# jwcalder/GraphLearningLayer

Measured on AMD Instinct MI355X. Metric: GLL fwd+bwd calls/sec (base=500,batch=500,d=512,k=10) at 1/2/4/8 GPU, higher is better.
Workload: dtype f32; 1 GPU; ns; base=500, batch=500, d=512, k=10, classes=10, parallelism=dp1, upstream_grad=fixed seeded dL/dU, autograd_thread=caller, collective=none

## Files before the change

graphlearninglayer_amd/_lib.py:

```python
from __future__ import annotations

import ctypes as ct
import os
import threading

HERE = os.path.dirname(os.path.abspath(__file__))
LIB_PATH = os.environ.get("GLL_LIB_PATH") or os.path.join(HERE, "libgll.so")

GLL_OK = 0
GLL_DT_F32, GLL_DT_F64, GLL_DT_I64 = 0, 1, 2
FLAG_CG_GRID = 1
FLAG_CG_PERCOL = 8
FLAG_DIAG_GRID_OVERSUB = 128
FLAG_DIAG_GRID_FAIL = 256
FLAG_CG_ELL = 512
FLAG_CG_VR = 1024
FLAG_GRAD_ROWS = 2048
FLAG_GRAD_CHUNK = 4096
FLAG_GRAM_INLINE = 8192
FLAG_BWD_UNFUSED = 16384
FLAG_KNN_PANEL = 65536
FLAG_D2_F32 = 131072
FLAG_ROW_ORDER_OFF = 262144
KNOB_VR_RV, KNOB_GRID_CAP, KNOB_GRAM_TILE, KNOB_SEL_FORM, KNOB_GRAM_TAIL, KNOB_ROW_PRE = 0, 1, 2, 3, 4, 5
ST_TINY_EPS, ST_FWD_NONCONV, ST_FWD_ITERS, ST_BWD_NONCONV, ST_BWD_ITERS = 0, 1, 2, 3, 4
ST_KNN_RESCAN = 5
ST_SOLVE_FAILED = 6
ST_GRID_RESCUED = 10
ST_KNN_MERGE = 7
ST_NWORDS = 16
K_GRAM, K_SELECT, K_FINALIZE, K_CG, K_EDGE, K_GRAD = range(6)
K_BWD = 6
K_PARAM = 7
K_LOSS = 8
K_COUNT = 9
PG_Y, PG_TAU, PG_EPS = 1, 2, 4
XT_F32, XT_F16, XT_BF16 = 0, 1, 2
UF_NORMALIZE = 1
MAX_D_FEATURES = 4096

EXPORTS = (
    "gll_workspace_bytes", "gll_forward", "gll_backward", "gll_forward_batched",
    "gll_backward_batched", "gll_param_grad_scratch_bytes", "gll_param_grad_batched",
    "gll_ce_head_scratch_bytes", "gll_ce_head_batched", "gll_margin_head_scratch_bytes",
    "gll_margin_head_batched", "gll_graph", "gll_workspace_view",
    "gll_cg_csr_workspace_bytes", "gll_cg_csr", "gll_prof_enable", "gll_prof_read",
    "gll_kernel_name", "gll_strerror", "gll_set_knob", "gll_build_id", "gll_select_route",
    "gll_workspace_solve_view", "gll_workspace_knn_view", "gll_gram_route",
    "gll_features_forward", "gll_features_backward", "gll_features_calls",
)


class Problem(ct.Structure):
    _fields_ = [
        ("n", ct.c_int32), ("d", ct.c_int32), ("base", ct.c_int32), ("C", ct.c_int32),
        ("K", ct.c_int32), ("max_iter", ct.c_int32), ("tau", ct.c_float), ("eps", ct.c_float),
        ("rtol", ct.c_float), ("flags", ct.c_int32), ("status_sink", ct.c_void_p),
    ]


class View(ct.Structure):
    _fields_ = [(name, ct.c_void_p) for name in (
        "knn_idx", "knn_d2", "eps", "row_start", "row_len", "col", "w", "d2", "deg", "U32",
        "wadj", "status")]
# ... 52 lines not shown
    lib.gll_workspace_knn_view.restype = i32
    lib.gll_gram_route.argtypes = [P, i32, i32, i32, ct.POINTER(ct.c_int32)]
    lib.gll_gram_route.restype = i32
    lib.gll_cg_csr_workspace_bytes.argtypes = [i32, i32]
    lib.gll_cg_csr_workspace_bytes.restype = sz
    lib.gll_cg_csr.argtypes = [i32, i32, vp, vp, vp, vp, vp, ct.c_float, i32, vp, vp, vp, vp]
    lib.gll_cg_csr.restype = i32
    lib.gll_prof_enable.argtypes = [i32, i32]
    lib.gll_prof_enable.restype = i32
    lib.gll_prof_read.argtypes = [i32, ct.POINTER(ct.c_double), ct.POINTER(ct.c_int)]
    lib.gll_prof_read.restype = i32
    lib.gll_kernel_name.argtypes = [i32]
    lib.gll_kernel_name.restype = ct.c_char_p
    lib.gll_select_route.argtypes = [ct.POINTER(Problem), i32, i32, i32, ct.POINTER(ct.c_int32)]
    lib.gll_select_route.restype = i32
    lib.gll_set_knob.argtypes = [i32, i32]
    lib.gll_set_knob.restype = i32
    lib.gll_strerror.argtypes = [i32]
    lib.gll_strerror.restype = ct.c_char_p
    lib.gll_build_id.argtypes = []
    lib.gll_build_id.restype = ct.c_char_p
    lib.gll_features_forward.argtypes = [ct.c_int64, ct.c_int32, vp, i32, i32, vp, vp, vp]
    lib.gll_features_forward.restype = i32
    lib.gll_features_backward.argtypes = [ct.c_int64, ct.c_int32, vp, vp, vp, i32, vp, i32, vp]
    lib.gll_features_backward.restype = i32
    lib.gll_features_calls.argtypes = []
    lib.gll_features_calls.restype = ct.c_int64
    return lib


# ... 39 lines not shown
```

graphlearninglayer_amd/csrc/api.hip:

```cpp
#include <atomic>
#include <cstdio>
#include <cstdlib>
#include <mutex>
#include <unordered_map>
#include <vector>

#include "knn_route.h"

namespace gll {

struct ProfState {
    int period[GLL_K_COUNT] = {};
    long count[GLL_K_COUNT] = {};
    bool on[GLL_K_COUNT] = {};
    std::vector<hipEvent_t> pending[GLL_K_COUNT];
    std::vector<hipEvent_t> pool;
    std::mutex mu;
    hipEvent_t get() {
        if (!pool.empty()) {
            hipEvent_t e = pool.back();
            pool.pop_back();
            return e;
        }
        hipEvent_t e;
// ... 202 lines not shown
    if (B < 1 || B > 65535) return GLL_ERR_INVALID_ARG;
    if (!X || !ws || !gradX || (p->n > p->base && !gbar)) return GLL_ERR_INVALID_ARG;
    if (g_dtype != GLL_DT_F32 && g_dtype != GLL_DT_F64) return GLL_ERR_INVALID_ARG;
    Layout L(*p);
    const Batch bt = make_batch(p, L, B, GLL_DT_F32, g_dtype);
    hipStream_t s = static_cast<hipStream_t>(stream);
    const float rtol = p->rtol > 0.f ? p->rtol : 1e-6f;
    const int max_iter = p->max_iter > 0 ? p->max_iter : 1000;
    int32_t* st = public_status(p, L, ws);
    float* wU = L.at<float>(ws, L.Wadj) + size_t(L.base) * L.C;
    const bool auto_eps = !(p->eps > 0.f);
    if (B == 1 && !auto_eps) {
        const hipError_t e = launch_cg_grad_fused(L, ws, gbar, g_dtype, X, p->eps, gradX, rtol,
                                                  max_iter, st + GLL_ST_BWD_NONCONV,
                                                  st + GLL_ST_BWD_ITERS, st + GLL_ST_SOLVE_FAILED,
                                                  vec_ok(X, p->d), s);
        if (e != hipErrorNotSupported) return hip_status(e);
    }
    hipError_t e = launch_cg_luu(L, bt, ws, gbar, bt.g, g_dtype, nullptr, wU, rtol, max_iter,
                                 st + GLL_ST_BWD_NONCONV, st + GLL_ST_BWD_ITERS,
                                 st + GLL_ST_SOLVE_FAILED, s);
    if (e != hipSuccess) return GLL_ERR_HIP;
    return hip_status(launch_backward_grad(L, bt, ws, X, auto_eps, p->eps, gradX,
                                           vec_ok(X, p->d), s));
}

}

using namespace gll;

extern "C" {
// ... 279 lines not shown
    if (rc != GLL_OK) return rc;
    if (B < 1 || B > 65535 || !out) return GLL_ERR_INVALID_ARG;
    Layout L(*p);
    if (L.PR < L.n ? (B > 1 || rows < 1 || rows > L.PR) : rows != L.n) return GLL_ERR_INVALID_ARG;
    Batch bt;
    bt.B = B;
    const SelRoute rt = select_route(L, bt, x_aligned && p->d % 4 == 0, 0, rows);
    const SelVariant& v = rt.v;
    const SelWideVariant& w = rt.w;
    const int32_t words[GLL_SEL_ROUTE_WORDS] = {
        rt.wide, rt.wide ? w.V : v.KC, rt.wide ? w.NP : v.V, rt.wide ? w.CAP : v.NP,
        rt.wide ? w.KMX : v.PG, rt.wide ? w.TOP : v.NU, v.XQ, v.R, v.CH, v.H,
        select_table_index(rt), select_table_rows()};
    for (int q = 0; q < GLL_SEL_ROUTE_WORDS; ++q) out[q] = words[q];
    return words[10] >= 0 ? GLL_OK : GLL_ERR_UNSUPPORTED;
}

#ifndef GLL_BUILD_ID
#define GLL_BUILD_ID "unknown"
#endif
const char* gll_build_id(void) { return GLL_BUILD_ID; }

const char* gll_strerror(int code) {
    switch (code) {
        case GLL_OK: return "ok";
        case GLL_ERR_INVALID_ARG: return "invalid argument";
        case GLL_ERR_UNSUPPORTED: return "unsupported problem size (see include/gll.h limits)";
        case GLL_ERR_HIP: return "HIP launch error";
        default: return "unknown error";
    }
// ... 69 lines not shown
```

graphlearninglayer_amd/csrc/gll_internal.h:

```cpp
#pragma once

#include <hip/hip_runtime.h>
#include <hip/hip_ext.h>
#include <stdint.h>
#include <stdlib.h>

#include <type_traits>

#include "gll.h"

namespace gll {

constexpr int kWave = 64;
constexpr int kMaxKm1 = 56;
constexpr int kMaxKm1Wide = 128;
constexpr int kMaxKm1Huge = 256;

constexpr int kStOvfCount = 8;
constexpr int kStBump = 9;
constexpr int kStPermValid = 11;
constexpr int kPiv = 64;
constexpr int kStWords = GLL_ST_NWORDS;

inline int ell_slots(int m) {
// ... 450 lines not shown
                              int max_iter, int32_t* st_nonconv, int32_t* st_iters,
                              int32_t* st_failed, hipStream_t s);
hipError_t launch_cg_grid_csr(int m, int C, const int32_t* row_ptr, const int32_t* col,
                              const float* val, int64_t nnz, const float* b, float* x,
                              float atol, int max_iter, int32_t* iters, int32_t* nonconv,
                              int32_t* failed, float* ws, hipStream_t s);
hipError_t launch_cg_csr(int m, int C, const int32_t* row_ptr, const int32_t* col,
                         const float* val, const float* b, float* x, float atol, int max_iter,
                         int32_t* iters, int32_t* nonconv, float* gvec, hipStream_t s);
hipError_t launch_backward_grad(const Layout& L, const Batch& bt, void* ws, const float* X,
                                bool auto_eps, float eps_fixed, float* gradX, bool vec,
                                hipStream_t s);
hipError_t launch_cg_grad_fused(const Layout& L, void* ws, const void* gbar, int g_dtype,
                                const float* X, float eps_fixed, float* gradX, float rtol,
                                int max_iter, int32_t* st_nonconv, int32_t* st_iters,
                                int32_t* st_failed, bool vec, hipStream_t s);
size_t param_grad_scratch_bytes(int n, int B);
hipError_t launch_param_grad(const Layout& L, int B, void* ws, float eps_fixed, int what,
                             float* gradY, double* grad_tau, double* grad_eps, void* scratch,
                             hipStream_t s);
size_t ce_head_scratch_bytes(int m, int B);
hipError_t launch_ce_head(const Layout& L, int B, void* ws, const int64_t* targets, double* loss,
                          float* gbar, double* row_loss, int64_t* pred_label, int64_t* correct,
                          void* scratch, hipStream_t s);
hipError_t launch_margin_head(const Layout& L, int B, void* ws, const int64_t* other, double* loss,
                              float* gbar, double* row_margin, int64_t* label, int64_t* second,
                              int64_t* moved, void* scratch, hipStream_t s);
hipError_t launch_unit_rows(int64_t rows, int d, const void* Z, int z_dtype, int flags, float* X,
                            float* rnorm, hipStream_t s);
hipError_t launch_unit_grad(int64_t rows, int d, const float* gX, const float* X,
                            const float* rnorm, int flags, void* gZ, int z_dtype, hipStream_t s);
// ... 4 lines not shown
```

graphlearninglayer_amd/csrc/solve.hip:

```cpp
#include <cstdio>
#include <cstdlib>
#include <mutex>
#include <unordered_set>

#include "gll_internal.h"
#include "grad_common.h"

namespace gll {

GLL_TRACE_UNIT(solve)
#ifdef GLL_TRACE
static __device__ unsigned long long g_fz[5 * 4096];
void trace_read_fz(unsigned long long* out) {
    (void)hipMemcpyFromSymbol(out, HIP_SYMBOL(g_fz), sizeof(g_fz));
}
#define GLL_FZ(slot, wv, val)                                                                  \
    do {                                                                                       \
        if (lane_id() == 0 && (wv) < 4096) g_fz[(slot) * 4096 + (wv)] = (val);                 \
    } while (0)
#else
#define GLL_FZ(slot, wv, val) do {} while (0)
#endif

static constexpr size_t kLdsLimit = 160 * 1024;
// ... 844 lines not shown
    if (cap > eu_bound) cap = eu_bound;
    if (cap > kOvfLds) cap = kOvfLds;
    if (cap < 0) cap = 0;
    lds += size_t(cap) * 8;
    if (S > ell_emit(L, bt.B)) return hipErrorInvalidValue;
    auto fn = cg_ell_kernel<NT, R, S, TB, MODE>;
    allow_full_lds(reinterpret_cast<const void*>(fn));
    launch_k(fn, dim3(L.C, bt.B), NT, lds, s,
        L.m, L.C, L.base, L.at<int32_t>(ws, L.row_start), L.at<int32_t>(ws, L.row_len),
        L.at<int32_t>(ws, L.ucnt), L.at<int32_t>(ws, L.col), L.at<float>(ws, L.w),
        L.at<float>(ws, L.diag), b, out64, out32, rtol, max_iter, int(cap), st_nonconv, st_iters,
        L.at<int4>(ws, L.ell), bt.ws, bs, bt.u, bt.st);
    return launch_status("solve.hip:run_ell");
}

struct EllCgArgs {
    int m, C, base;
    const int32_t* row_start;
    const int32_t* row_len;
    const int32_t* ucnt;
    const int32_t* col;
    const float* wv;
    const float* diag;
    const void* b;
    float* out32;
    float rtol;
    int max_iter, mat_cap;
    int32_t* st_nonconv;
    int32_t* st_iters;
    const int4* ell;
};

template <int NT, int S, typename TB, int ND>
__global__ __launch_bounds__(NT) void cg_grad_fused_kernel(EllCgArgs c, EdgeArgs a,
                                                           const float* __restrict__ X,
                                                           float* __restrict__ out,
                                                           unsigned* fsync, int32_t* st_failed) {
    const int C = c.C;
    if (int(blockIdx.x) < C) {
        cg_ell_body<NT, 1, S, TB, 3>(int2{int(blockIdx.x), 0}, fsync, c.m, C, c.base,
                                     c.row_start, c.row_len, c.ucnt, c.col, c.wv, c.diag,
                                     static_cast<const TB*>(c.b), nullptr, c.out32, c.rtol,
                                     c.max_iter, c.mat_cap, c.st_nonconv, c.st_iters, c.ell,
                                     0, 0, 0, 0);
        return;
    }
    constexpr int NC = 10;
    constexpr int EB = ND <= 2 ? 16 : 8;
    __shared__ int s_ok;
    const int lane = lane_id();
    int i0;
    {
        extern __shared__ __attribute__((aligned(16))) float smem[];
        int* srt = reinterpret_cast<int*>(smem);
        int* crk = srt + a.n;
        const int nch = (a.n + kWave - 1) / kWave;
        int* cnt = crk + a.n;
        constexpr int NW = NT / kWave;
        const int w = threadIdx.x >> 6;
        for (int q = w; q < nch; q += NW) {
            const int i = q * kWave + lane;
            int cls = -1;
            if (i < a.n) {
                float bv = -3.0e38f;
                cls = 0;
#pragma unroll
// ... 19 lines not shown
            for (int kk = 0; kk < k; ++kk)
                for (int q = 0; q < nch; ++q) before += cnt[q * NC + kk];
            for (int q = 0; q < nch; ++q) {
                const int c0 = cnt[q * NC + k];
                cnt[q * NC + k] = before;
                before += c0;
            }
        }
        __syncthreads();
        for (int i = threadIdx.x; i < a.n; i += NT) {
            const int v = crk[i];
            srt[cnt[(i / kWave) * NC + (v >> 16)] + (v & 0xffff)] = i;
        }
        __syncthreads();
        const int G = int(gridDim.x) - C, b = int(blockIdx.x), x = b & 7;
        int ord = 0;
#pragma unroll
        for (int xx = 0; xx < 8; ++xx) {
            const int f = C + ((xx - C % 8 + 8) & 7);
            const int cx = f < C + G ? (C + G - 1 - f) / 8 + 1 : 0;
            if (xx < x) ord += cx;
        }
        ord += (b - (C + ((x - C % 8 + 8) & 7))) >> 3;
        const int pos = ord * NW + w;
        i0 = pos < a.n ? srt[pos] : a.n;
    }
    const bool live = i0 < a.n;
    const int i = live ? i0 : 0;
    const int d = a.d;
    const int beg = a.row_start[i];
    const int end = live ? beg + a.row_len[i] : beg;
    const float ei = a.eps_fixed;
    const float* xi = X + size_t(i) * d;
    f32x4 xv[ND];
#pragma unroll
    for (int q = 0; q < ND; ++q) xv[q] = load4_raw<true>(xi, 4 * lane + 4 * kWave * q, d);
    typedef float f32x2 __attribute__((ext_vector_type(2)));
    float pi[NC];
#pragma unroll
    for (int q = 0; q < NC; q += 2) {
        const f32x2 v = *reinterpret_cast<const f32x2*>(a.P + size_t(i) * NC + q);
        pi[q] = v.x, pi[q + 1] = v.y;
    }
    const __amdgpu_buffer_rsrc_t rw =
        __builtin_amdgcn_make_buffer_rsrc(const_cast<float*>(a.Wadj), 0, a.n * NC * 4, 0x00020000);
    auto edge_pre = [&](int e, int& cj, float& we, float* pj) {
        const bool el = e < end;
        cj = el ? a.col[e] : i;
        we = el ? a.w[e] : 0.f;
#pragma unroll
        for (int q = 0; q < NC; q += 2) {
            const f32x2 v = *reinterpret_cast<const f32x2*>(a.P + size_t(cj) * NC + q);
// ... 10 lines not shown
        float g = 0.f;
#pragma unroll
        for (int q = 0; q < NC; ++q) g = __builtin_fmaf(wi[q] - wj[q], pj[q] - pi[q], g);
        const float ej = a.eps_fixed;
        const float v = -8.f * we / (ei * ej);
        return e < end ? g * v : 0.f;
    };
    int cj;
    float we, pj[NC];
    edge_pre(beg + lane, cj, we, pj);
    const int cnt0 = min(kWave, end - beg);
#ifdef GLL_TRACE
    const bool tr = int(blockIdx.x) == C && threadIdx.x == 0;
    if (tr) g_trace[16] = __builtin_amdgcn_s_memrealtime();
#endif
    f32x4 v[EB][ND];
#pragma unroll
    for (int u = 0; u < EB; ++u) {
        const int t = u < cnt0 ? u : 0;
        const float* xj = X + size_t(readlane_i(cj, t)) * d;
#pragma unroll
        for (int q = 0; q < ND; ++q) v[u][q] = load4_raw<true>(xj, 4 * lane + 4 * kWave * q, d);
    }
    if (threadIdx.x == 0) {
        int ok = __hip_atomic_load(fsync + 64, __ATOMIC_RELAXED, __HIP_MEMORY_SCOPE_AGENT) == 0u;
        unsigned spins = 0;
        const unsigned long long t0 = wall_ticks();
        while (ok && __hip_atomic_load(fsync + 96, __ATOMIC_RELAXED, __HIP_MEMORY_SCOPE_AGENT) ==
               0u) {
            __builtin_amdgcn_s_sleep(2);
            if ((++spins & 15u) == 0 && wall_ticks() - t0 > kWaitTicks) {
                ok = 0;
                break;
            }
        }
        s_ok = ok;
    }
    __syncthreads();
    const bool ok = s_ok != 0;
#ifdef GLL_TRACE
    if (tr) g_trace[17] = __builtin_amdgcn_s_memrealtime();
    GLL_FZ(0, i0, __builtin_amdgcn_s_memrealtime());
#endif
#pragma unroll
    for (int q = 0; q < NC; ++q)
        wi[q] = __builtin_bit_cast(
            float, __builtin_amdgcn_raw_buffer_load_b32(rw, (i * NC + q) * 4, 0, kSc1W));
    f32x4 acc[ND];
#pragma unroll
    for (int q = 0; q < ND; ++q) acc[q] = f32x4{0.f, 0.f, 0.f, 0.f};
    for (int e0 = beg; e0 < end; e0 += kWave) {
        if (e0 != beg) edge_pre(e0 + lane, cj, we, pj);
        const float cf = edge_coef(e0 + lane, cj, we, pj);
#ifdef GLL_TRACE
        if (e0 == beg) {
            float cfo = cf;
            asm volatile("s_waitcnt vmcnt(0)" : "+v"(cfo)::"memory");
            if (cfo == 12345.f) g_trace[9] = 0;
            GLL_FZ(1, i0, __builtin_amdgcn_s_memrealtime());
        }
#endif
        const int cnt = min(kWave, end - e0);
        for (int t0 = 0; t0 < cnt; t0 += EB) {
            float sv[EB];
            if (e0 != beg || t0 != 0) {
#pragma unroll
                for (int u = 0; u < EB; ++u) {
                    const int t = t0 + u < cnt ? t0 + u : t0;
                    const float* xj = X + size_t(readlane_i(cj, t)) * d;
#pragma unroll
                    for (int q = 0; q < ND; ++q) v[u][q] = load4_raw<true>(xj, 4 * lane + 4 * kWave * q, d);
                }
            }
#pragma unroll
            for (int u = 0; u < EB; ++u) {
                const int t = t0 + u < cnt ? t0 + u : t0;
                sv[u] = t0 + u < cnt ? readlane_f(cf, t) : 0.f;
            }
#pragma unroll
            for (int u = 0; u < EB; ++u) {
#pragma unroll
                for (int q = 0; q < ND; ++q) acc[q] += sv[u] * (xv[q] - v[u][q]);
            }
        }
    }
#ifdef GLL_TRACE
    {
        f32x4 ao = acc[0];
        asm volatile("" : "+v"(ao));
        if (ao.x == 12345.f) g_trace[9] = 0;
        GLL_FZ(2, i0, __builtin_amdgcn_s_memrealtime());
    }
#endif
    if (live) {
        const float nanf_ = __builtin_nanf("");
        float* oi = out + size_t(i) * d;
#pragma unroll
        for (int q = 0; q < ND; ++q) {
            const int k = 4 * lane + 4 * kWave * q;
            const f32x4 r = ok ? acc[q] : f32x4{nanf_, nanf_, nanf_, nanf_};
            if (k < d) __builtin_nontemporal_store(r, reinterpret_cast<f32x4*>(oi + k));
        }
    }
#ifdef GLL_TRACE
    asm volatile("s_waitcnt vmcnt(0)" ::: "memory");
    GLL_FZ(3, i0, __builtin_amdgcn_s_memrealtime());
    {
        unsigned hw;
        asm volatile("s_getreg_b32 %0, hwreg(HW_REG_HW_ID)" : "=s"(hw));
        unsigned xcc;
        asm volatile("s_getreg_b32 %0, hwreg(HW_REG_XCC_ID)" : "=s"(xcc));
        GLL_FZ(4, i0, (unsigned long long)(end - beg) | ((unsigned long long)((hw >> 8) & 0xffff) << 16) |
                          ((unsigned long long)(xcc & 0xff) << 40));
    }
#endif
    __syncthreads();
#ifdef GLL_TRACE
    if (tr) g_trace[18] = __builtin_amdgcn_s_memrealtime();
    if (threadIdx.x == 0) atomicMax(&g_trace[19], __builtin_amdgcn_s_memrealtime());
#endif
    if (threadIdx.x == 0) {
        if (!ok) {
            __hip_atomic_fetch_or(fsync + 64, 1u, __ATOMIC_RELAXED, __HIP_MEMORY_SCOPE_AGENT);
            if (st_failed) atomicOr(st_failed, 1);
            asm volatile("s_waitcnt vmcnt(0)" ::: "memory");
        }
        const unsigned ng = gridDim.x - unsigned(C);
        const unsigned old = __hip_atomic_fetch_add(fsync + 32, 1u, __ATOMIC_RELAXED,
                                                    __HIP_MEMORY_SCOPE_AGENT);
        if (old + 1u == ng &&
            __hip_atomic_load(fsync + 64, __ATOMIC_RELAXED, __HIP_MEMORY_SCOPE_AGENT) == 0u) {
            __hip_atomic_store(fsync, 0u, __ATOMIC_RELAXED, __HIP_MEMORY_SCOPE_AGENT);
            __hip_atomic_store(fsync + 32, 0u, __ATOMIC_RELAXED, __HIP_MEMORY_SCOPE_AGENT);
            __hip_atomic_store(fsync + 96, 0u, __ATOMIC_RELAXED, __HIP_MEMORY_SCOPE_AGENT);
        }
    }
}

template <int NT, int ND, typename TB>
static hipError_t run_fused(const Layout& L, void* ws, const TB* b, const float* X,
                            float eps_fixed, float* gradX, float rtol, int max_iter,
                            int32_t* st_nonconv, int32_t* st_iters, int32_t* st_failed,
                            hipStream_t s) {
    constexpr int S = 24;
    size_t lds = 128 * 4 + size_t((L.m + 3) & ~3) * 4 * 2;
    const int64_t eu_bound = int64_t(L.m + L.n) * (L.K - 1);
    int64_t cap = int64_t(kLdsDyn - lds) / 8;
    if (cap > eu_bound) cap = eu_bound;
    if (cap < 0) cap = 0;
    lds += size_t(cap) * 8;
    const size_t sort_lds = size_t(L.n) * 8 + size_t((L.n + kWave - 1) / kWave) * 10 * 4;
    if (sort_lds > kLdsDyn) return hipErrorNotSupported;
    if (lds < sort_lds) lds = sort_lds;
    auto fn = cg_grad_fused_kernel<NT, S, TB, ND>;
    allow_full_lds(reinterpret_cast<const void*>(fn));
    const int G = L.C + (L.n + NT / kWave - 1) / (NT / kWave);
    const int nb = occupancy_blocks(reinterpret_cast<const void*>(fn), NT, lds);
    if (int64_t(nb) * device_cus() < G) return hipErrorNotSupported;
    EllCgArgs c;
    c.m = L.m;
    c.C = L.C;
    c.base = L.base;
    c.row_start = L.at<int32_t>(ws, L.row_start);
    c.row_len = L.at<int32_t>(ws, L.row_len);
    c.ucnt = L.at<int32_t>(ws, L.ucnt);
    c.col = L.at<int32_t>(ws, L.col);
    c.wv = L.at<float>(ws, L.w);
    c.diag = L.at<float>(ws, L.diag);
    c.b = b;
    c.out32 = L.at<float>(ws, L.Wadj) + size_t(L.base) * L.C;
    c.rtol = rtol;
    c.max_iter = max_iter;
    c.mat_cap = int(cap);
    c.st_nonconv = st_nonconv;
    c.st_iters = st_iters;
    c.ell = L.at<int4>(ws, L.ell);
    const EdgeArgs a = make_edge_args(L, 0, ws, eps_fixed);
    prof_begin(GLL_K_BWD, s);
    launch_k(fn, dim3(unsigned(G)), NT, lds, s, c, a, X, gradX, L.at<unsigned>(ws, L.fsync),
             st_failed);
    prof_end(GLL_K_BWD, s);
    return launch_status("solve.hip:run_fused");
}

hipError_t launch_cg_grad_fused(const Layout& L, void* ws, const void* gbar, int g_dtype,
                                const float* X, float eps_fixed, float* gradX, float rtol,
                                int max_iter, int32_t* st_nonconv, int32_t* st_iters,
                                int32_t* st_failed, bool vec, hipStream_t s) {
    const int m = L.m;
    if (L.C != 10 || !(eps_fixed > 0.f) || !vec || m < 1 || m > 512 || L.RV != 0 ||
        ell_emit(L, 1) != 24 || L.d > 1024)
        return hipErrorNotSupported;
    if (L.flags & (GLL_FLAG_BWD_UNFUSED | GLL_FLAG_CG_GRID | GLL_FLAG_GRAD_CHUNK))
        return hipErrorNotSupported;
    if (size_t(L.n) * L.d * 4 > (size_t(4) << 20)) return hipErrorNotSupported;
    const int nd = (L.d + 255) / 256;
#define GLL_FUSED(NT_)                                                                       \
    {                                                                                        \
        if (g_dtype == GLL_DT_F32) {                                                         \
            const float* b = static_cast<const float*>(gbar);                                \
            if (nd <= 1) return run_fused<NT_, 1>(L, ws, b, X, eps_fixed, gradX, rtol, max_iter, st_nonconv, st_iters, st_failed, s); \
            if (nd <= 2) return run_fused<NT_, 2>(L, ws, b, X, eps_fixed, gradX, rtol, max_iter, st_nonconv, st_iters, st_failed, s); \
            return run_fused<NT_, 4>(L, ws, b, X, eps_fixed, gradX, rtol, max_iter, st_nonconv, st_iters, st_failed, s); \
        }                                                                                    \
        const double* b = static_cast<const double*>(gbar);                                  \
        if (nd <= 1) return run_fused<NT_, 1>(L, ws, b, X, eps_fixed, gradX, rtol, max_iter, st_nonconv, st_iters, st_failed, s); \
        if (nd <= 2) return run_fused<NT_, 2>(L, ws, b, X, eps_fixed, gradX, rtol, max_iter, st_nonconv, st_iters, st_failed, s); \
        return run_fused<NT_, 4>(L, ws, b, X, eps_fixed, gradX, rtol, max_iter, st_nonconv, st_iters, st_failed, s); \
    }
    if (m <= 64) GLL_FUSED(64);
    if (m <= 128) GLL_FUSED(128);
    if (m <= 256) GLL_FUSED(256);
    GLL_FUSED(512);
#undef GLL_FUSED
}

template <int NT, int R, int RV, typename TB>
static hipError_t run_vr(const Layout& L, const Batch& bt, void* ws, const TB* b, size_t bs,
                         double* out64, float* out32, float rtol, int max_iter,
                         int32_t* st_nonconv, int32_t* st_iters, hipStream_t s) {
    if (L.m > NT * R || L.RV != RV || L.VRM <= 0 || L.VRM > 63) {
        (void)hipGetLastError();
        return hipErrorInvalidValue;
    }
    const size_t mp4 = size_t((L.m + 3) & ~3);
    const size_t lds = 128 * 4 + mp4 * 4 + (size_t(NT) * RV + 4 * mp4) * 4 +
                       size_t(NT) * RV * 4 + mp4 * 4;
// ... 170 lines not shown
```

include/gll.h:

```cpp
#ifndef GLL_H
#define GLL_H

#include <stddef.h>
#include <stdint.h>

#ifdef __cplusplus
extern "C" {
#endif

#define GLL_OK 0
#define GLL_ERR_INVALID_ARG (-1)
#define GLL_ERR_UNSUPPORTED (-2)
#define GLL_ERR_HIP (-3)

#define GLL_DT_F32 0
#define GLL_DT_F64 1
#define GLL_DT_I64 2

#define GLL_ST_TINY_EPS 0
#define GLL_ST_FWD_NONCONV 1
#define GLL_ST_FWD_ITERS 2
#define GLL_ST_BWD_NONCONV 3
#define GLL_ST_BWD_ITERS 4
#define GLL_ST_KNN_RESCAN 5
#define GLL_ST_SOLVE_FAILED 6
#define GLL_ST_KNN_MERGE 7
#define GLL_ST_GRID_RESCUED 10
#define GLL_ST_NWORDS 16

#define GLL_FLAG_CG_GRID 1
#define GLL_FLAG_CG_PERCOL 8
#define GLL_FLAG_DIAG_GRID_OVERSUB 128
#define GLL_FLAG_DIAG_GRID_FAIL 256
#define GLL_FLAG_CG_ELL 512
#define GLL_FLAG_CG_VR 1024
#define GLL_FLAG_GRAD_ROWS 2048
#define GLL_FLAG_GRAD_CHUNK 4096
#define GLL_FLAG_GRAM_INLINE 8192
#define GLL_FLAG_BWD_UNFUSED 16384
#define GLL_FLAG_KNN_PANEL 65536
#define GLL_FLAG_D2_F32 131072
#define GLL_FLAG_ROW_ORDER_OFF 262144
#define GLL_FLAG_ALL (1 | 8 | 128 | 256 | 512 | 1024 | 2048 | 4096 | 8192 | 16384 | 65536 | \
                      131072 | 262144)

#define GLL_KNOB_VR_RV 0
#define GLL_KNOB_GRID_CAP 1
#define GLL_KNOB_GRAM_TILE 2
#define GLL_KNOB_SEL_FORM 3
#define GLL_KNOB_GRAM_TAIL 4
#define GLL_KNOB_ROW_PRE 5
#define GLL_KNOB_COUNT 6
int gll_set_knob(int knob, int value);

typedef struct gll_problem {
    int32_t n;
    int32_t d;
    int32_t base;
    int32_t C;
    int32_t K;
    int32_t max_iter;
    float tau;
    float eps;
    float rtol;
    int32_t flags;
    int32_t* status_sink;
} gll_problem;
// ... 96 lines not shown
#define GLL_K_CG 3
#define GLL_K_EDGE 4
#define GLL_K_GRAD 5
#define GLL_K_BWD 6
#define GLL_K_PARAM 7
#define GLL_K_LOSS 8
#define GLL_K_COUNT 9
int gll_prof_enable(int kid, int period);
int gll_prof_read(int kid, double* ms_total, int* count);
const char* gll_kernel_name(int kid);

#define GLL_SEL_ROUTE_WORDS 12
int gll_select_route(const gll_problem* p, int B, int x_aligned, int rows,
                     int32_t out[GLL_SEL_ROUTE_WORDS]);

const char* gll_build_id(void);

const char* gll_strerror(int code);

#define GLL_XT_F32 0
#define GLL_XT_F16 1
#define GLL_XT_BF16 2
#define GLL_UF_NORMALIZE 1
int gll_features_forward(int64_t rows, int32_t d, const void* Z, int z_dtype, int flags,
                         float* X, float* rnorm, void* stream);
int gll_features_backward(int64_t rows, int32_t d, const float* gX, const float* X,
                          const float* rnorm, int flags, void* gZ, int z_dtype, void* stream);
int64_t gll_features_calls(void);

#ifdef __cplusplus
// ... 4 lines not shown
```

Before: 16230 calls/s.

## Split long gradient rows across multiple waves in fused CG-grad kernel

The fused CG+gradient kernel can now split a row's feature dimension into 2 or 4 parts when the row has many edges, so one row is handled by several waves. The grid grows (up to twice the row count) to supply those waves, with a prefix-sum assignment of work items to waves. Extra waves exit early through a counter that keeps the sync-reset logic working. The aim is better load balance and more memory-level parallelism for the edge gather. The cost is larger launches, more prefix-scan work per block, and duplicated per-row coefficient work.

```diff
diff --git a/graphlearninglayer_amd/_lib.py b/graphlearninglayer_amd/_lib.py
--- a/graphlearninglayer_amd/_lib.py
+++ b/graphlearninglayer_amd/_lib.py
@@ -23,11 +23,13 @@
 FLAG_D2_F32 = 131072
 FLAG_ROW_ORDER_OFF = 262144
 KNOB_VR_RV, KNOB_GRID_CAP, KNOB_GRAM_TILE, KNOB_SEL_FORM, KNOB_GRAM_TAIL, KNOB_ROW_PRE = 0, 1, 2, 3, 4, 5
+KNOB_GRAD_SPLIT = 6
 ST_TINY_EPS, ST_FWD_NONCONV, ST_FWD_ITERS, ST_BWD_NONCONV, ST_BWD_ITERS = 0, 1, 2, 3, 4
 ST_KNN_RESCAN = 5
 ST_SOLVE_FAILED = 6
 ST_GRID_RESCUED = 10
 ST_KNN_MERGE = 7
+ST_GRAD_SPLIT = 12
 ST_NWORDS = 16
 K_GRAM, K_SELECT, K_FINALIZE, K_CG, K_EDGE, K_GRAD = range(6)
 K_BWD = 6
@@ -47,7 +49,7 @@
     "gll_cg_csr_workspace_bytes", "gll_cg_csr", "gll_prof_enable", "gll_prof_read",
     "gll_kernel_name", "gll_strerror", "gll_set_knob", "gll_build_id", "gll_select_route",
     "gll_workspace_solve_view", "gll_workspace_knn_view", "gll_gram_route",
-    "gll_features_forward", "gll_features_backward", "gll_features_calls",
+    "gll_features_forward", "gll_features_backward", "gll_features_calls", "gll_fused_plan",
 )
 
 
@@ -130,6 +132,8 @@
     lib.gll_kernel_name.restype = ct.c_char_p
     lib.gll_select_route.argtypes = [ct.POINTER(Problem), i32, i32, i32, ct.POINTER(ct.c_int32)]
     lib.gll_select_route.restype = i32
+    lib.gll_fused_plan.argtypes = [ct.POINTER(Problem), i32, i32, ct.POINTER(ct.c_int32)]
+    lib.gll_fused_plan.restype = i32
     lib.gll_set_knob.argtypes = [i32, i32]
     lib.gll_set_knob.restype = i32
     lib.gll_strerror.argtypes = [i32]
diff --git a/graphlearninglayer_amd/csrc/api.hip b/graphlearninglayer_amd/csrc/api.hip
--- a/graphlearninglayer_amd/csrc/api.hip
+++ b/graphlearninglayer_amd/csrc/api.hip
@@ -240,7 +240,7 @@
         const hipError_t e = launch_cg_grad_fused(L, ws, gbar, g_dtype, X, p->eps, gradX, rtol,
                                                   max_iter, st + GLL_ST_BWD_NONCONV,
                                                   st + GLL_ST_BWD_ITERS, st + GLL_ST_SOLVE_FAILED,
-                                                  vec_ok(X, p->d), s);
+                                                  st + GLL_ST_GRAD_SPLIT, vec_ok(X, p->d), s);
         if (e != hipErrorNotSupported) return hip_status(e);
     }
     hipError_t e = launch_cg_luu(L, bt, ws, gbar, bt.g, g_dtype, nullptr, wU, rtol, max_iter,
@@ -550,6 +550,19 @@
         select_table_index(rt), select_table_rows()};
     for (int q = 0; q < GLL_SEL_ROUTE_WORDS; ++q) out[q] = words[q];
     return words[10] >= 0 ? GLL_OK : GLL_ERR_UNSUPPORTED;
+}
+
+int gll_fused_plan(const gll_problem* p, int x_aligned, int capacity,
+                   int32_t out[GLL_FUSED_PLAN_WORDS]) {
+    int rc = check(p);
+    if (rc != GLL_OK) return rc;
+    if (!out) return GLL_ERR_INVALID_ARG;
+    Layout L(*p);
+    if (capacity < 0)
+        return fused_plan_device(L, p->eps, x_aligned && p->d % 4 == 0, GLL_DT_F64, out)
+                   ? GLL_OK : GLL_ERR_UNSUPPORTED;
+    return fused_plan(L, p->eps, x_aligned && p->d % 4 == 0, capacity, out) ? GLL_OK
+                                                                             : GLL_ERR_UNSUPPORTED;
 }
 
 #ifndef GLL_BUILD_ID
diff --git a/graphlearninglayer_amd/csrc/gll_internal.h b/graphlearninglayer_amd/csrc/gll_internal.h
--- a/graphlearninglayer_amd/csrc/gll_internal.h
+++ b/graphlearninglayer_amd/csrc/gll_internal.h
@@ -488,7 +488,9 @@
 hipError_t launch_cg_grad_fused(const Layout& L, void* ws, const void* gbar, int g_dtype,
                                 const float* X, float eps_fixed, float* gradX, float rtol,
                                 int max_iter, int32_t* st_nonconv, int32_t* st_iters,
-                                int32_t* st_failed, bool vec, hipStream_t s);
+                                int32_t* st_failed, int32_t* st_split, bool vec, hipStream_t s);
+bool fused_plan(const Layout& L, float eps_fixed, bool vec, int64_t capacity, int32_t out[8]);
+bool fused_plan_device(const Layout& L, float eps_fixed, bool vec, int g_dtype, int32_t out[8]);
 size_t param_grad_scratch_bytes(int n, int B);
 hipError_t launch_param_grad(const Layout& L, int B, void* ws, float eps_fixed, int what,
                              float* gradY, double* grad_tau, double* grad_eps, void* scratch,
diff --git a/graphlearninglayer_amd/csrc/solve.hip b/graphlearninglayer_amd/csrc/solve.hip
--- a/graphlearninglayer_amd/csrc/solve.hip
+++ b/graphlearninglayer_amd/csrc/solve.hip
@@ -882,6 +882,69 @@
     return launch_status("solve.hip:run_ell");
 }
 
+struct FusedPlan {
+    int nt, nd;
+    int grid;
+    int base_grid;
+    int waves;
+    int split;
+    size_t lds;
+    int64_t mat_cap;
+};
+
+__host__ __device__ inline int row_parts(int len, int eb, int pmax) {
+    const int l = len < kWave ? len : kWave;
+    int p = 1;
+    while (p < pmax && l > eb * p) p *= 2;
+    return p;
+}
+__host__ __device__ constexpr int max_parts(int nd) { return nd >= 2 ? 4 : 1; }
+__host__ __device__ constexpr int fused_eb(int nd) { return nd <= 2 ? 16 : 8; }
+
+template <int W> struct PartVec { typedef f32x4 type; };
+template <> struct PartVec<2> { typedef f32x2 type; };
+template <int W>
+__device__ __forceinline__ typename PartVec<W>::type part_load(const float* __restrict__ p, int k,
+                                                               int lim) {
+    return *reinterpret_cast<const typename PartVec<W>::type*>(p + (k < lim ? k : 0));
+}
+template <int NV, int W>
+__device__ __forceinline__ void part_load_row(typename PartVec<W>::type* r,
+                                              const float* __restrict__ x, int fo, int lane, int d) {
+#pragma unroll
+    for (int q = 0; q < NV; ++q) r[q] = part_load<W>(x, fo + W * lane + W * kWave * q, d);
+}
+
+template <int S, int NV, int W>
+__device__ __forceinline__ void part_gather(typename PartVec<W>::type* v,
+                                            const float* __restrict__ X, int cj, int t0, int cnt,
+                                            int fo, int lane, int d) {
+#pragma unroll
+    for (int u = 0; u < S; ++u) {
+        const int t = t0 + u < cnt ? t0 + u : t0;
+        part_load_row<NV, W>(v + u * NV, X + size_t(readlane_i(cj, t)) * d, fo, lane, d);
+    }
+}
+
+template <int S, int NV, int W, bool FIRST>
+__device__ __forceinline__ void part_fma(typename PartVec<W>::type* acc,
+                                         const typename PartVec<W>::type* xv,
+                                         const typename PartVec<W>::type* v, float cf, int t0) {
+    static_assert(kWave % S == 0, "slots divide the 64 edges of a pass");
+    constexpr int SB = S < 16 ? S : 16;
+#pragma unroll
+    for (int u0 = 0; u0 < S; u0 += SB) {
+        float sv[SB];
+#pragma unroll
+        for (int u = 0; u < SB; ++u) sv[u] = readlane_f(cf, FIRST ? u0 + u : t0 + u0 + u);
+#pragma unroll
+        for (int u = 0; u < SB; ++u) {
+#pragma unroll
+            for (int q = 0; q < NV; ++q) acc[q] += sv[u] * (xv[q] - v[(u0 + u) * NV + q]);
+        }
+    }
+}
+
 struct EllCgArgs {
     int m, C, base;
     const int32_t* row_start;
@@ -903,7 +966,8 @@
 __global__ __launch_bounds__(NT) void cg_grad_fused_kernel(EllCgArgs c, EdgeArgs a,
                                                            const float* __restrict__ X,
                                                            float* __restrict__ out,
-                                                           unsigned* fsync, int32_t* st_failed) {
+                                                           unsigned* fsync, int32_t* st_failed,
+                                                           int32_t* st_split, int split) {
     const int C = c.C;
     if (int(blockIdx.x) < C) {
         cg_ell_body<NT, 1, S, TB, 3>(int2{int(blockIdx.x), 0}, fsync, c.m, C, c.base,
@@ -917,7 +981,20 @@
     constexpr int EB = ND <= 2 ? 16 : 8;
     __shared__ int s_ok;
     const int lane = lane_id();
-    int i0;
+    auto exit_count = [&]() {
+        const unsigned ng = gridDim.x - unsigned(C);
+        const unsigned old = __hip_atomic_fetch_add(fsync + 32, 1u, __ATOMIC_RELAXED,
+                                                    __HIP_MEMORY_SCOPE_AGENT);
+        if (old + 1u == ng &&
+            __hip_atomic_load(fsync + 64, __ATOMIC_RELAXED, __HIP_MEMORY_SCOPE_AGENT) == 0u) {
+            __hip_atomic_store(fsync, 0u, __ATOMIC_RELAXED, __HIP_MEMORY_SCOPE_AGENT);
+            __hip_atomic_store(fsync + 32, 0u, __ATOMIC_RELAXED, __HIP_MEMORY_SCOPE_AGENT);
+            __hip_atomic_store(fsync + 96, 0u, __ATOMIC_RELAXED, __HIP_MEMORY_SCOPE_AGENT);
+        }
+    };
+    constexpr int PMAX = max_parts(ND);
+    int i0, pos;
+    int part = 0, nparts = 1;
     {
         extern __shared__ __attribute__((aligned(16))) float smem[];
         int* srt = reinterpret_cast<int*>(smem);
@@ -967,16 +1044,87 @@
         }
         __syncthreads();
         const int G = int(gridDim.x) - C, b = int(blockIdx.x), x = b & 7;
-        int ord = 0;
-#pragma unroll
-        for (int xx = 0; xx < 8; ++xx) {
-            const int f = C + ((xx - C % 8 + 8) & 7);
-            const int cx = f < C + G ? (C + G - 1 - f) / 8 + 1 : 0;
-            if (xx < x) ord += cx;
-        }
-        ord += (b - (C + ((x - C % 8 + 8) & 7))) >> 3;
-        const int pos = ord * NW + w;
+        auto xcd_rank = [&](int act) -> int {
+            const int j = (b - (C + ((x - C % 8 + 8) & 7))) >> 3;
+            int ord = 0, all = 0, tot = 0, mine = 0;
+#pragma unroll
+            for (int xx = 0; xx < 8; ++xx) {
+                const int f = C + ((xx - C % 8 + 8) & 7);
+                const int cx = f < C + G ? (C + G - 1 - f) / 8 + 1 : 0;
+                const int ax = min(cx, act / 8 + (xx < act % 8 ? 1 : 0));
+                if (xx < x) ord += ax, all += cx;
+                if (xx == x) mine = ax;
+                tot += ax;
+            }
+            if (tot < act) return all + j;
+            return j < mine ? ord + j : -1;
+        };
+        pos = xcd_rank(G) * NW + w;
         i0 = pos < a.n ? srt[pos] : a.n;
+        int nsplit = 0;
+        int wrank = 0;
+        if (PMAX > 1 && split) {
+            int* ipre = crk;
+            int* coff = cnt;
+            for (int q = w; q < nch; q += NW) {
+                const int r = q * kWave + lane;
+                const int p = r < a.n ? row_parts(a.row_len[srt[r]], EB, PMAX) : 0;
+                int inc = p;
+#pragma unroll
+                for (int off = 1; off < kWave; off <<= 1) {
+                    const int t = __shfl_up(inc, off);
+                    if (lane >= off) inc += t;
+                }
+                if (r < a.n) ipre[r] = ((inc - p) << 3) | p;
+                const uint64_t ms = __ballot(p > 1);
+                if (lane == kWave - 1) coff[q] = inc, coff[nch + q] = __popcll(ms);
+            }
+            __syncthreads();
+            if (threadIdx.x == 0) {
+                int items = 0, rows = 0;
+                for (int q = 0; q < nch; ++q) {
+                    const int c0 = coff[q];
+                    coff[q] = items;
+                    items += c0;
+                    rows += coff[nch + q];
+                }
+                coff[2 * nch] = items;
+                coff[2 * nch + 1] = rows;
+            }
+            __syncthreads();
+            const int items = coff[2 * nch];
+            if (items <= G * NW) {
+                nsplit = coff[2 * nch + 1];
+                i0 = a.n;
+                wrank = xcd_rank((items + NW - 1) / NW);
+                pos = wrank * NW + w;
+                if (wrank >= 0 && pos < items) {
+                    int cq = 0;
+                    for (int q0 = 0; q0 < nch; q0 += kWave) {
+                        const int q = q0 + lane;
+                        cq += __popcll(__ballot(q < nch && coff[q] <= pos));
+                    }
+                    const int r = (cq - 1) * kWave + lane;
+                    const int e = r < a.n ? ipre[r] : 0;
+                    const int first = coff[cq - 1] + (e >> 3);
+                    const uint64_t hit = __ballot((e & 7) != 0 && pos >= first && pos < first + (e & 7));
+                    if (hit != 0) {
+                        const int l = __ffsll((unsigned long long)hit) - 1;
+                        i0 = srt[(cq - 1) * kWave + l];
+                        nparts = readlane_i(e & 7, l);
+                        part = pos - readlane_i(first, l);
+                    }
+                }
+            }
+        }
+        if (int(blockIdx.x) == C && threadIdx.x == 0 && st_split) *st_split = nsplit;
+        if (wrank < 0) {
+            if (threadIdx.x == 0) exit_count();
+            return;
+        }
+        nparts = __builtin_amdgcn_readfirstlane(nparts);
+        part = __builtin_amdgcn_readfirstlane(part);
+        i0 = __builtin_amdgcn_readfirstlane(i0);
     }
     const bool live = i0 < a.n;
     const int i = live ? i0 : 0;
@@ -985,10 +1133,16 @@
     const int end = live ? beg + a.row_len[i] : beg;
     const float ei = a.eps_fixed;
     const float* xi = X + size_t(i) * d;
-    f32x4 xv[ND];
-#pragma unroll
-    for (int q = 0; q < ND; ++q) xv[q] = load4_raw<true>(xi, 4 * lane + 4 * kWave * q, d);
-    typedef float f32x2 __attribute__((ext_vector_type(2)));
+    const int fo = part * (4 * kWave * ND / nparts);
+    auto by_part = [&](auto f) {
+        if constexpr (PMAX > 1) {
+            if (nparts == 2) return f(std::integral_constant<int, ND / 2>{}, std::integral_constant<int, 4>{});
+            if (nparts == 4)
+                return f(std::integral_constant<int, (ND >= 4 ? ND / 4 : 1)>{},
+                         std::integral_constant<int, (ND >= 4 ? 4 : 2)>{});
+        }
+        return f(std::integral_constant<int, ND>{}, std::integral_constant<int, 4>{});
+    };
     float pi[NC];
 #pragma unroll
     for (int q = 0; q < NC; q += 2) {
@@ -1029,106 +1183,98 @@
     const bool tr = int(blockIdx.x) == C && threadIdx.x == 0;
     if (tr) g_trace[16] = __builtin_amdgcn_s_memrealtime();
 #endif
-    f32x4 v[EB][ND];
-#pragma unroll
-    for (int u = 0; u < EB; ++u) {
-        const int t = u < cnt0 ? u : 0;
-        const float* xj = X + size_t(readlane_i(cj, t)) * d;
-#pragma unroll
-        for (int q = 0; q < ND; ++q) v[u][q] = load4_raw<true>(xj, 4 * lane + 4 * kWave * q, d);
-    }
-    if (threadIdx.x == 0) {
-        int ok = __hip_atomic_load(fsync + 64, __ATOMIC_RELAXED, __HIP_MEMORY_SCOPE_AGENT) == 0u;
-        unsigned spins = 0;
-        const unsigned long long t0 = wall_ticks();
-        while (ok && __hip_atomic_load(fsync + 96, __ATOMIC_RELAXED, __HIP_MEMORY_SCOPE_AGENT) ==
-               0u) {
-            __builtin_amdgcn_s_sleep(2);
-            if ((++spins & 15u) == 0 && wall_ticks() - t0 > kWaitTicks) {
-                ok = 0;
-                break;
-            }
-        }
-        s_ok = ok;
-    }
-    __syncthreads();
-    const bool ok = s_ok != 0;
+    auto wait_release = [&]() -> bool {
+        if (threadIdx.x == 0) {
+            int ok = __hip_atomic_load(fsync + 64, __ATOMIC_RELAXED, __HIP_MEMORY_SCOPE_AGENT) == 0u;
+            unsigned spins = 0;
+            const unsigned long long t0 = wall_ticks();
+            while (ok && __hip_atomic_load(fsync + 96, __ATOMIC_RELAXED,
+                                           __HIP_MEMORY_SCOPE_AGENT) == 0u) {
+                __builtin_amdgcn_s_sleep(2);
+                if ((++spins & 15u) == 0 && wall_ticks() - t0 > kWaitTicks) {
+                    ok = 0;
+                    break;
+                }
+            }
+            s_ok = ok;
+        }
+        __syncthreads();
+        return s_ok != 0;
+    };
+    bool ok = false;
+    if (!live) ok = wait_release();
+    else by_part([&](auto nv, auto wd) {
+        constexpr int NV = nv(), W = wd();
+        constexpr int SL = EB * ND * 4 / (NV * W);
+        typedef typename PartVec<W>::type VT;
+        VT xv[NV];
+        part_load_row<NV, W>(xv, xi, fo, lane, d);
+        VT v[SL * NV];
+        part_gather<SL, NV, W>(v, X, cj, 0, cnt0, fo, lane, d);
+        ok = wait_release();
 #ifdef GLL_TRACE
-    if (tr) g_trace[17] = __builtin_amdgcn_s_memrealtime();
-    GLL_FZ(0, i0, __builtin_amdgcn_s_memrealtime());
+        if (tr) g_trace[17] = __builtin_amdgcn_s_memrealtime();
+        const int fzi = live ? pos : 4096;
+        GLL_FZ(0, fzi, __builtin_amdgcn_s_memrealtime());
 #endif
 #pragma unroll
-    for (int q = 0; q < NC; ++q)
-        wi[q] = __builtin_bit_cast(
-            float, __builtin_amdgcn_raw_buffer_load_b32(rw, (i * NC + q) * 4, 0, kSc1W));
-    f32x4 acc[ND];
-#pragma unroll
-    for (int q = 0; q < ND; ++q) acc[q] = f32x4{0.f, 0.f, 0.f, 0.f};
-    for (int e0 = beg; e0 < end; e0 += kWave) {
-        if (e0 != beg) edge_pre(e0 + lane, cj, we, pj);
-        const float cf = edge_coef(e0 + lane, cj, we, pj);
+        for (int q = 0; q < NC; ++q)
+            wi[q] = __builtin_bit_cast(
+                float, __builtin_amdgcn_raw_buffer_load_b32(rw, (i * NC + q) * 4, 0, kSc1W));
+        VT acc[NV];
+#pragma unroll
+        for (int q = 0; q < NV; ++q) acc[q] = VT(0.f);
+        for (int e0 = beg; e0 < end; e0 += kWave) {
+            if (e0 != beg) edge_pre(e0 + lane, cj, we, pj);
+            const float cf = edge_coef(e0 + lane, cj, we, pj);
 #ifdef GLL_TRACE
-        if (e0 == beg) {
-            float cfo = cf;
-            asm volatile("s_waitcnt vmcnt(0)" : "+v"(cfo)::"memory");
-            if (cfo == 12345.f) g_trace[9] = 0;
-            GLL_FZ(1, i0, __builtin_amdgcn_s_memrealtime());
-        }
+            if (e0 == beg) {
+                float cfo = cf;
+                asm volatile("s_waitcnt vmcnt(0)" : "+v"(cfo)::"memory");
+                if (cfo == 12345.f) g_trace[9] = 0;
+                GLL_FZ(1, fzi, __builtin_amdgcn_s_memrealtime());
+            }
 #endif
-        const int cnt = min(kWave, end - e0);
-        for (int t0 = 0; t0 < cnt; t0 += EB) {
-            float sv[EB];
-            if (e0 != beg || t0 != 0) {
-#pragma unroll
-                for (int u = 0; u < EB; ++u) {
-                    const int t = t0 + u < cnt ? t0 + u : t0;
-                    const float* xj = X + size_t(readlane_i(cj, t)) * d;
-#pragma unroll
-                    for (int q = 0; q < ND; ++q) v[u][q] = load4_raw<true>(xj, 4 * lane + 4 * kWave * q, d);
-                }
-            }
-#pragma unroll
-            for (int u = 0; u < EB; ++u) {
-                const int t = t0 + u < cnt ? t0 + u : t0;
-                sv[u] = t0 + u < cnt ? readlane_f(cf, t) : 0.f;
-            }
-#pragma unroll
-            for (int u = 0; u < EB; ++u) {
-#pragma unroll
-                for (int q = 0; q < ND; ++q) acc[q] += sv[u] * (xv[q] - v[u][q]);
-            }
-        }
-    }
+            const int cnt = min(kWave, end - e0);
+            if (e0 != beg) part_gather<SL, NV, W>(v, X, cj, 0, cnt, fo, lane, d);
+            part_fma<SL, NV, W, true>(acc, xv, v, cf, 0);
+            for (int t0 = SL; t0 < cnt; t0 += SL) {
+                part_gather<SL, NV, W>(v, X, cj, t0, cnt, fo, lane, d);
+                part_fma<SL, NV, W, false>(acc, xv, v, cf, t0);
+            }
+        }
 #ifdef GLL_TRACE
-    {
-        f32x4 ao = acc[0];
-        asm volatile("" : "+v"(ao));
-        if (ao.x == 12345.f) g_trace[9] = 0;
-        GLL_FZ(2, i0, __builtin_amdgcn_s_memrealtime());
-    }
+        {
+            VT ao = acc[0];
+            asm volatile("" : "+v"(ao));
+            if (ao.x == 12345.f) g_trace[9] = 0;
+            GLL_FZ(2, fzi, __builtin_amdgcn_s_memrealtime());
+        }
 #endif
-    if (live) {
-        const float nanf_ = __builtin_nanf("");
-        float* oi = out + size_t(i) * d;
-#pragma unroll
-        for (int q = 0; q < ND; ++q) {
-            const int k = 4 * lane + 4 * kWave * q;
-            const f32x4 r = ok ? acc[q] : f32x4{nanf_, nanf_, nanf_, nanf_};
-            if (k < d) __builtin_nontemporal_store(r, reinterpret_cast<f32x4*>(oi + k));
-        }
-    }
+        if (live) {
+            const float nanf_ = __builtin_nanf("");
+            float* oi = out + size_t(i) * d;
+#pragma unroll
+            for (int q = 0; q < NV; ++q) {
+                const int k = fo + W * lane + W * kWave * q;
+                const VT r = ok ? acc[q] : VT(nanf_);
+                if (k < d) __builtin_nontemporal_store(r, reinterpret_cast<VT*>(oi + k));
+            }
+        }
 #ifdef GLL_TRACE
-    asm volatile("s_waitcnt vmcnt(0)" ::: "memory");
-    GLL_FZ(3, i0, __builtin_amdgcn_s_memrealtime());
-    {
-        unsigned hw;
-        asm volatile("s_getreg_b32 %0, hwreg(HW_REG_HW_ID)" : "=s"(hw));
-        unsigned xcc;
-        asm volatile("s_getreg_b32 %0, hwreg(HW_REG_XCC_ID)" : "=s"(xcc));
-        GLL_FZ(4, i0, (unsigned long long)(end - beg) | ((unsigned long long)((hw >> 8) & 0xffff) << 16) |
-                          ((unsigned long long)(xcc & 0xff) << 40));
-    }
+        asm volatile("s_waitcnt vmcnt(0)" ::: "memory");
+        GLL_FZ(3, fzi, __builtin_amdgcn_s_memrealtime());
+        {
+            unsigned hw;
+            asm volatile("s_getreg_b32 %0, hwreg(HW_REG_HW_ID)" : "=s"(hw));
+            unsigned xcc;
+            asm volatile("s_getreg_b32 %0, hwreg(HW_REG_XCC_ID)" : "=s"(xcc));
+            GLL_FZ(4, fzi, (unsigned long long)(end - beg) | ((unsigned long long)((hw >> 8) & 0xffff) << 16) |
+                               ((unsigned long long)(xcc & 0xff) << 40) |
+                               ((unsigned long long)(i & 0xfff) << 48) | (1ull << 63));
+        }
 #endif
+    });
     __syncthreads();
 #ifdef GLL_TRACE
     if (tr) g_trace[18] = __builtin_amdgcn_s_memrealtime();
@@ -1140,24 +1286,11 @@
             if (st_failed) atomicOr(st_failed, 1);
             asm volatile("s_waitcnt vmcnt(0)" ::: "memory");
         }
-        const unsigned ng = gridDim.x - unsigned(C);
-        const unsigned old = __hip_atomic_fetch_add(fsync + 32, 1u, __ATOMIC_RELAXED,
-                                                    __HIP_MEMORY_SCOPE_AGENT);
-        if (old + 1u == ng &&
-            __hip_atomic_load(fsync + 64, __ATOMIC_RELAXED, __HIP_MEMORY_SCOPE_AGENT) == 0u) {
-            __hip_atomic_store(fsync, 0u, __ATOMIC_RELAXED, __HIP_MEMORY_SCOPE_AGENT);
-            __hip_atomic_store(fsync + 32, 0u, __ATOMIC_RELAXED, __HIP_MEMORY_SCOPE_AGENT);
-            __hip_atomic_store(fsync + 96, 0u, __ATOMIC_RELAXED, __HIP_MEMORY_SCOPE_AGENT);
-        }
-    }
-}
-
-template <int NT, int ND, typename TB>
-static hipError_t run_fused(const Layout& L, void* ws, const TB* b, const float* X,
-                            float eps_fixed, float* gradX, float rtol, int max_iter,
-                            int32_t* st_nonconv, int32_t* st_iters, int32_t* st_failed,
-                            hipStream_t s) {
-    constexpr int S = 24;
+        exit_count();
+    }
+}
+
+static bool fused_lds(const Layout& L, int nt, int nd, FusedPlan* pl) {
     size_t lds = 128 * 4 + size_t((L.m + 3) & ~3) * 4 * 2;
     const int64_t eu_bound = int64_t(L.m + L.n) * (L.K - 1);
     int64_t cap = int64_t(kLdsDyn - lds) / 8;
@@ -1165,13 +1298,90 @@
     if (cap < 0) cap = 0;
     lds += size_t(cap) * 8;
     const size_t sort_lds = size_t(L.n) * 8 + size_t((L.n + kWave - 1) / kWave) * 10 * 4;
-    if (sort_lds > kLdsDyn) return hipErrorNotSupported;
+    if (sort_lds > kLdsDyn) return false;
     if (lds < sort_lds) lds = sort_lds;
+    pl->nt = nt;
+    pl->nd = nd;
+    pl->lds = lds;
+    pl->mat_cap = cap;
+    return true;
+}
+static bool fused_grid(const Layout& L, int64_t capacity, FusedPlan* pl) {
+    const int nw = pl->nt / kWave;
+    pl->base_grid = L.C + (L.n + nw - 1) / nw;
+    if (capacity < pl->base_grid) return false;
+    pl->split = max_parts(pl->nd) > 1 && knob(GLL_KNOB_GRAD_SPLIT) != 2;
+    int64_t g = pl->base_grid;
+    if (pl->split) g = std::min<int64_t>(capacity, L.C + (2 * int64_t(L.n) + nw - 1) / nw);
+    pl->grid = int(g);
+    pl->waves = (pl->grid - L.C) * nw;
+    return true;
+}
+static bool fused_shape(const Layout& L, float eps_fixed, bool vec, int* nt, int* nd) {
+    const int m = L.m;
+    if (L.C != 10 || !(eps_fixed > 0.f) || !vec || m < 1 || m > 512 || L.RV != 0 ||
+        ell_emit(L, 1) != 24 || L.d > 1024)
+        return false;
+    if (L.flags & (GLL_FLAG_BWD_UNFUSED | GLL_FLAG_CG_GRID | GLL_FLAG_GRAD_CHUNK)) return false;
+    if (size_t(L.n) * L.d * 4 > (size_t(4) << 20)) return false;
+    *nd = L.d <= 256 ? 1 : (L.d <= 512 ? 2 : 4);
+    *nt = m <= 64 ? 64 : (m <= 128 ? 128 : (m <= 256 ? 256 : 512));
+    return true;
+}
+static void fused_plan_words(const Layout& L, const FusedPlan& pl, int32_t out[8]) {
+    out[0] = pl.nt, out[1] = pl.nd, out[2] = pl.grid, out[3] = pl.base_grid, out[4] = pl.waves;
+    out[5] = pl.waves - L.n, out[6] = pl.split, out[7] = int32_t(pl.lds);
+}
+bool fused_plan(const Layout& L, float eps_fixed, bool vec, int64_t capacity, int32_t out[8]) {
+    FusedPlan pl;
+    int nt, nd;
+    if (!fused_shape(L, eps_fixed, vec, &nt, &nd) || !fused_lds(L, nt, nd, &pl) ||
+        !fused_grid(L, capacity, &pl))
+        return false;
+    fused_plan_words(L, pl, out);
+    return true;
+}
+
+template <int NT, int ND, typename TB>
+static const void* fused_fn() {
+    return reinterpret_cast<const void*>(cg_grad_fused_kernel<NT, 24, TB, ND>);
+}
+template <int NT, typename TB>
+static const void* fused_fn_nd(int nd) {
+    return nd <= 1 ? fused_fn<NT, 1, TB>() : (nd <= 2 ? fused_fn<NT, 2, TB>() : fused_fn<NT, 4, TB>());
+}
+template <typename TB>
+static const void* fused_fn_nt(int nt, int nd) {
+    return nt == 64 ? fused_fn_nd<64, TB>(nd)
+                    : (nt == 128 ? fused_fn_nd<128, TB>(nd)
+                                 : (nt == 256 ? fused_fn_nd<256, TB>(nd) : fused_fn_nd<512, TB>(nd)));
+}
+bool fused_plan_device(const Layout& L, float eps_fixed, bool vec, int g_dtype, int32_t out[8]) {
+    FusedPlan pl;
+    int nt, nd;
+    if (!fused_shape(L, eps_fixed, vec, &nt, &nd) || !fused_lds(L, nt, nd, &pl)) return false;
+    const void* fn = g_dtype == GLL_DT_F32 ? fused_fn_nt<float>(nt, nd) : fused_fn_nt<double>(nt, nd);
+    allow_full_lds(fn);
+    if (!fused_grid(L, int64_t(occupancy_blocks(fn, nt, pl.lds)) * device_cus(), &pl)) return false;
+    fused_plan_words(L, pl, out);
+    return true;
+}
+
+template <int NT, int ND, typename TB>
+static hipError_t run_fused(const Layout& L, void* ws, const TB* b, const float* X,
+                            float eps_fixed, float* gradX, float rtol, int max_iter,
+                            int32_t* st_nonconv, int32_t* st_iters, int32_t* st_failed,
+                            int32_t* st_split, hipStream_t s) {
+    constexpr int S = 24;
+    FusedPlan pl;
+    if (!fused_lds(L, NT, ND, &pl)) return hipErrorNotSupported;
+    const size_t lds = pl.lds;
+    const int64_t cap = pl.mat_cap;
     auto fn = cg_grad_fused_kernel<NT, S, TB, ND>;
     allow_full_lds(reinterpret_cast<const void*>(fn));
-    const int G = L.C + (L.n + NT / kWave - 1) / (NT / kWave);
     const int nb = occupancy_blocks(reinterpret_cast<const void*>(fn), NT, lds);
-    if (int64_t(nb) * device_cus() < G) return hipErrorNotSupported;
+    if (!fused_grid(L, int64_t(nb) * device_cus(), &pl)) return hipErrorNotSupported;
+    const int G = pl.grid;
     EllCgArgs c;
     c.m = L.m;
     c.C = L.C;
@@ -1193,7 +1403,7 @@
     const EdgeArgs a = make_edge_args(L, 0, ws, eps_fixed);
     prof_begin(GLL_K_BWD, s);
     launch_k(fn, dim3(unsigned(G)), NT, lds, s, c, a, X, gradX, L.at<unsigned>(ws, L.fsync),
-             st_failed);
+             st_failed, st_split, pl.split);
     prof_end(GLL_K_BWD, s);
     return launch_status("solve.hip:run_fused");
 }
@@ -1201,31 +1411,25 @@
 hipError_t launch_cg_grad_fused(const Layout& L, void* ws, const void* gbar, int g_dtype,
                                 const float* X, float eps_fixed, float* gradX, float rtol,
                                 int max_iter, int32_t* st_nonconv, int32_t* st_iters,
-                                int32_t* st_failed, bool vec, hipStream_t s) {
-    const int m = L.m;
-    if (L.C != 10 || !(eps_fixed > 0.f) || !vec || m < 1 || m > 512 || L.RV != 0 ||
-        ell_emit(L, 1) != 24 || L.d > 1024)
-        return hipErrorNotSupported;
-    if (L.flags & (GLL_FLAG_BWD_UNFUSED | GLL_FLAG_CG_GRID | GLL_FLAG_GRAD_CHUNK))
-        return hipErrorNotSupported;
-    if (size_t(L.n) * L.d * 4 > (size_t(4) << 20)) return hipErrorNotSupported;
-    const int nd = (L.d + 255) / 256;
+                                int32_t* st_failed, int32_t* st_split, bool vec, hipStream_t s) {
+    int nt, nd;
+    if (!fused_shape(L, eps_fixed, vec, &nt, &nd)) return hipErrorNotSupported;
 #define GLL_FUSED(NT_)                                                                       \
     {                                                                                        \
         if (g_dtype == GLL_DT_F32) {                                                         \
             const float* b = static_cast<const float*>(gbar);                                \
-            if (nd <= 1) return run_fused<NT_, 1>(L, ws, b, X, eps_fixed, gradX, rtol, max_iter, st_nonconv, st_iters, st_failed, s); \
-            if (nd <= 2) return run_fused<NT_, 2>(L, ws, b, X, eps_fixed, gradX, rtol, max_iter, st_nonconv, st_iters, st_failed, s); \
-            return run_fused<NT_, 4>(L, ws, b, X, eps_fixed, gradX, rtol, max_iter, st_nonconv, st_iters, st_failed, s); \
+            if (nd <= 1) return run_fused<NT_, 1>(L, ws, b, X, eps_fixed, gradX, rtol, max_iter, st_nonconv, st_iters, st_failed, st_split, s); \
+            if (nd <= 2) return run_fused<NT_, 2>(L, ws, b, X, eps_fixed, gradX, rtol, max_iter, st_nonconv, st_iters, st_failed, st_split, s); \
+            return run_fused<NT_, 4>(L, ws, b, X, eps_fixed, gradX, rtol, max_iter, st_nonconv, st_iters, st_failed, st_split, s); \
         }                                                                                    \
         const double* b = static_cast<const double*>(gbar);                                  \
-        if (nd <= 1) return run_fused<NT_, 1>(L, ws, b, X, eps_fixed, gradX, rtol, max_iter, st_nonconv, st_iters, st_failed, s); \
-        if (nd <= 2) return run_fused<NT_, 2>(L, ws, b, X, eps_fixed, gradX, rtol, max_iter, st_nonconv, st_iters, st_failed, s); \
-        return run_fused<NT_, 4>(L, ws, b, X, eps_fixed, gradX, rtol, max_iter, st_nonconv, st_iters, st_failed, s); \
-    }
-    if (m <= 64) GLL_FUSED(64);
-    if (m <= 128) GLL_FUSED(128);
-    if (m <= 256) GLL_FUSED(256);
+        if (nd <= 1) return run_fused<NT_, 1>(L, ws, b, X, eps_fixed, gradX, rtol, max_iter, st_nonconv, st_iters, st_failed, st_split, s); \
+        if (nd <= 2) return run_fused<NT_, 2>(L, ws, b, X, eps_fixed, gradX, rtol, max_iter, st_nonconv, st_iters, st_failed, st_split, s); \
+        return run_fused<NT_, 4>(L, ws, b, X, eps_fixed, gradX, rtol, max_iter, st_nonconv, st_iters, st_failed, st_split, s); \
+    }
+    if (nt == 64) GLL_FUSED(64);
+    if (nt == 128) GLL_FUSED(128);
+    if (nt == 256) GLL_FUSED(256);
     GLL_FUSED(512);
 #undef GLL_FUSED
 }
diff --git a/include/gll.h b/include/gll.h
--- a/include/gll.h
+++ b/include/gll.h
@@ -26,6 +26,7 @@
 #define GLL_ST_SOLVE_FAILED 6
 #define GLL_ST_KNN_MERGE 7
 #define GLL_ST_GRID_RESCUED 10
+#define GLL_ST_GRAD_SPLIT 12
 #define GLL_ST_NWORDS 16
 
 #define GLL_FLAG_CG_GRID 1
@@ -50,7 +51,8 @@
 #define GLL_KNOB_SEL_FORM 3
 #define GLL_KNOB_GRAM_TAIL 4
 #define GLL_KNOB_ROW_PRE 5
-#define GLL_KNOB_COUNT 6
+#define GLL_KNOB_GRAD_SPLIT 6
+#define GLL_KNOB_COUNT 7
 int gll_set_knob(int knob, int value);
 
 typedef struct gll_problem {
@@ -177,6 +179,10 @@
 int gll_select_route(const gll_problem* p, int B, int x_aligned, int rows,
                      int32_t out[GLL_SEL_ROUTE_WORDS]);
 
+#define GLL_FUSED_PLAN_WORDS 8
+int gll_fused_plan(const gll_problem* p, int x_aligned, int capacity,
+                   int32_t out[GLL_FUSED_PLAN_WORDS]);
+
 const char* gll_build_id(void);
 
 const char* gll_strerror(int code);
```

Measured after the change: 16480 calls/s (median of 6 runs). 1.5% higher.
